# dohlee/metheor

Measured on AMD Instinct MI355X. Metric: M reads/sec (PDR+LPMD, 150bp WGBS), higher is better.
Workload: dtype u32; 1 GPU; S-chr19-10M (BASELINE config 2): 10000000 x 150bp reads/GPU, chr19 58.6 Mbp, 2.94 CpG calls/read, fused PDR+LPMD, reference CLI defaults; reads_per_gpu=10000000, cpg_calls_per_gpu=29424182, sites_emitted=726028, parallelism=contig-sharded x1

## Files before the change

### metheor_amd/build.py

```python
import hashlib
import json
import os
import shutil
import subprocess
import sys
import time

HERE = os.path.dirname(os.path.abspath(__file__))
CSRC = os.path.join(HERE, "csrc")
LIB = os.path.join(HERE, "libmetheor_hip.so")
ARCH = "gfx950"
HIP_FLAGS = os.environ.get("MTH_EXTRA_HIPFLAGS", "").split() + ["-O3", "-std=c++17", "-fPIC", "-Wall", "-ffp-contract=off", "-Wno-unused-result"]

HIP_SOURCES = ["mth_api.hip", "mth_pdr_lpmd.hip", "mth_pdr_wide.hip", "mth_quartet.hip", "mth_scan.hip", "mth_sites.hip", "mth_mhl_tile.hip", "mth_fdrp.hip", "mth_fdrp_wtile.hip", "mth_pairs.hip", "mth_decode.hip", "mth_sort.hip", "mth_fileorder.hip", "mth_inflate.hip", "mth_rccl.hip", "mth_tag.hip", "mth_multi.hip"]
HOST_LIB = os.path.join(HERE, "libmetheor_host.so")
HOST_SOURCES = [os.path.join("host", "bam_reader.cpp"), os.path.join("host", "host_api.cpp"),
                os.path.join("host", "parallel_decode.cpp"), os.path.join("host", "synth_bam.cpp"), os.path.join("host", "bai_index.cpp"), os.path.join("host", "sam_text.cpp")]
HOST_HEADERS = [os.path.join("host", "bam_reader.h"), os.path.join("host", "parallel_decode.h"), os.path.join("host", "bai_internal.h"), os.path.join("host", "sam_text.h"), os.path.join("..", "..", "include", "metheor_host.h")]
HEADERS = ["mth_common.h", "mth_ctx.h", "mth_quartet_dev.h", "mth_scan.h", "mth_tile_dev.h", "mth_wave_tile.h", os.path.join("..", "..", "include", "metheor_hip.h")]


def _hipcc():
    for c in (shutil.which("hipcc"), "/opt/rocm/bin/hipcc"):
        if c and os.path.exists(c):
            return c
    raise RuntimeError("hipcc not found: the engine is HIP-only (no CPU fallback)")


BUILD_INFO = os.path.join(HERE, "BUILD_INFO.json")


def _sha(path):
    with open(path, "rb") as f:
        return hashlib.sha256(f.read()).hexdigest()[:16]


def _stale(target, deps):
    if not os.path.exists(target):
        return True
    t = os.path.getmtime(target)
    return any(os.path.getmtime(d) > t for d in deps if os.path.exists(d))


def source_files():
    out = [os.path.join("csrc", s) for s in HIP_SOURCES + HEADERS + HOST_SOURCES + HOST_HEADERS] + [os.path.join("csrc", "host", "cli_main.cpp")]
    return sorted(set(os.path.normpath(p) for p in out))


def source_hashes():
    return {p: _sha(os.path.join(HERE, p)) for p in source_files()}


def _write_build_info(rebuilt):
    try:
        ver = subprocess.run([_hipcc(), "--version"], capture_output=True, text=True).stdout.splitlines()[0]
    except Exception:
        ver = "?"
    info = {"built_at": time.strftime("%Y-%m-%dT%H:%M:%SZ", time.gmtime()), "rebuilt_this_call": bool(rebuilt), "arch": ARCH, "hipcc": ver,
            "hip_flags": HIP_FLAGS, "artefacts": {os.path.basename(p): _sha(p) for p in (LIB, HOST_LIB, CLI) if os.path.exists(p)},
            "sources": source_hashes()}
    old = None
    if os.path.exists(BUILD_INFO):
        try:
            old = json.load(open(BUILD_INFO))
        except Exception:
            old = None
    if old and not rebuilt and old.get("sources") == info["sources"] and old.get("artefacts") == info["artefacts"]:
        return
    with open(BUILD_INFO, "w") as f:
        json.dump(info, f, indent=1, sort_keys=True)


# ... 72 lines not shown
```

### metheor_amd/csrc/mth_pdr_lpmd.hip

```cpp
#include "mth_ctx.h"
#include "mth_tile_dev.h"

#ifndef MTH_TILE_PF
#define MTH_TILE_PF 1
#endif

namespace mth {


constexpr int IDX_GROUPS = 1;
template <int NIDX>
__global__ __launch_bounds__(BLOCK) void k_build_index(const int32_t *__restrict__ read_start,
                                                       uint32_t n_reads, int32_t idx_base, int32_t idx_base2, int qshift,
                                                       uint32_t nq, int aligned16,
                                                       uint32_t *__restrict__ idx, uint32_t *__restrict__ idx2,
                                                       DevState *__restrict__ st, DevState *__restrict__ cst,
                                                       unsigned long long *__restrict__ bucket_sums, uint32_t n_bucket_words,
                                                       const uint32_t *__restrict__ cpg_off, uint32_t n_cpgs) {
    const uint32_t gtid = blockIdx.x * BLOCK + threadIdx.x;
    if (gtid == 0 && cst) cst->cur_base = cst->n_sites;
    for (uint32_t w = gtid; w < n_bucket_words; w += gridDim.x * BLOCK) bucket_sums[w] = 0ull;
    if (cpg_off && gtid < 64) {
        uint32_t best = 0;
#pragma unroll
// ... 266 lines not shown
    int32_t s = 0;
    uint32_t o0 = 0, n = 0, mq = 0;
    constexpr bool PF = MTH_TILE_PF && !CLAMP && sizeof(RelT) == 1 && NB == 8;
    uint32_t o1 = 0;
    if (PF) { if (i < hi) { o0 = a.cpg_off[i]; o1 = a.cpg_off[i + 1]; } }
    else if (i < hi) { s = a.read_start[i]; o0 = a.cpg_off[i]; n = a.cpg_off[i + 1] - o0; mq = a.read_mapq[i]; }
    while (i < hi) {
        const uint32_t inext = i + B;
        const bool more = inext < hi;
        uint32_t v[NB];
        int32_t r[NB];
        uint32_t rraw0 = 0, rraw1 = 0;
        uint32_t o0n = 0, o1n = 0;
        if constexpr (PF) {
            n = o1 - o0;
            const uint32_t *__restrict__ cp = a.cpg_pos + o0;
#pragma unroll
            for (int k4 = 0; k4 < NB / 4; ++k4) {
                const u32x4_a4 x = *reinterpret_cast<const u32x4_a4 *>(cp + 4 * k4);
                v[4 * k4] = x.x; v[4 * k4 + 1] = x.y; v[4 * k4 + 2] = x.z; v[4 * k4 + 3] = x.w;
            }
            if (do_lp) { const u32x2_a1 x = *reinterpret_cast<const u32x2_a1 *>(reinterpret_cast<const RelT *>(a.cpg_rel) + o0); rraw0 = x.x; rraw1 = x.y; }
            s = a.read_start[i]; mq = a.read_mapq[i];
            if (more) { o0n = a.cpg_off[inext]; o1n = a.cpg_off[inext + 1]; }
        }
        const bool owned = (s >= T0) && (s < T1);
        const bool lp_ok = do_lp && owned && (mq >= a.lpmd_min_qual);
        if (do_lp && owned) { n_read += 1; n_valid += lp_ok ? 1u : 0u; }
        const bool pdr_ok = a.want_pdr && (n >= a.min_cpgs) && (mq >= a.pdr_min_qual) && (n > 0);
        const bool work = (lp_ok || pdr_ok) && n != 0;
        const int32_t maxd = PACKED ? min(a.max_dist, 255) : min(a.max_dist, 1 << 20);
        const int32_t mind = max(a.min_dist, 0);
        const bool any_lp = maxd >= a.min_dist && maxd >= 0 && __any(work && lp_ok && n > 1);
        if (work) {
            const uint32_t *__restrict__ cp = a.cpg_pos + o0;
            const RelT *__restrict__ rp = rel + o0;
            if (PF) {
                (void)cp; (void)rp;
            } else if (!CLAMP) {
#pragma unroll
                for (int k4 = 0; k4 < NB / 4; ++k4) {
                    const u32x4_a4 x = *reinterpret_cast<const u32x4_a4 *>(cp + 4 * k4);
                    v[4 * k4] = x.x; v[4 * k4 + 1] = x.y; v[4 * k4 + 2] = x.z; v[4 * k4 + 3] = x.w;
                }
                if (any_lp) {
                    if constexpr (PACKED) { const u32x2_a1 x = *reinterpret_cast<const u32x2_a1 *>(rp); rraw0 = x.x; rraw1 = x.y; }
                    else load_rel<RelT, NB>(rp, r);
                }
            } else {
#pragma unroll
                for (int k = 0; k < NB; ++k) v[k] = cp[min((uint32_t)k, n - 1)];
                if (any_lp) {
#pragma unroll
                    for (int k = 0; k < NB; ++k) r[k] = (int32_t)rp[min((uint32_t)k, n - 1)];
                }
            }
        const uint32_t sm1 = (uint32_t)(s - 1);
        const uint32_t dead_w = ((MARGIN ? (uint32_t)(P0 - MG + (tid & 63)) : (uint32_t)T0 + (1u << 28)) & 0x7fffffffu) | (v[0] & 0x80000000u);
        const uint32_t n_lp = lp_ok ? min(n, (uint32_t)NB) : 0u;
        uint32_t acc = 0, xmax = (v[0] & 0x7fffffffu) - sm1;
        if constexpr (PACKED) {
            const uint32_t nrow = min(n, 8u);
            const uint4 ma = reinterpret_cast<const uint4 *>(&tabs.mtab[nrow][0])[0], mb = reinterpret_cast<const uint4 *>(&tabs.mtab[nrow][0])[1];
            const uint32_t mk[8] = {ma.x, ma.y, ma.z, ma.w, mb.x, mb.y, mb.z, mb.w};
            uint32_t xs[8];
            xs[0] = xmax;
#pragma unroll
            for (int k = 1; k < 8; ++k) {
                xs[k] = __builtin_amdgcn_bitop3_b32(v[k] - sm1, mk[k], 0x7fffffffu, 0x80);
                v[k] = __builtin_amdgcn_bitop3_b32(v[k], dead_w, mk[k], 0xe4);
                acc = __builtin_amdgcn_bitop3_b32(acc, v[k], v[0], 0xf6);
            }
            xmax = max(max(max(xs[0], xs[1]), max(xs[2], xs[3])), max(max(xs[4], xs[5]), max(xs[6], xs[7])));
        } else {
#pragma unroll
            for (int k = 1; k < NB; ++k) {
                const bool live = (uint32_t)k < n;
                const uint32_t x = (v[k] & 0x7fffffffu) - sm1;
                xmax = max(xmax, live ? x : 0u);
                v[k] = live ? v[k] : dead_w;
                acc |= v[k] ^ v[0];
            }
            if (any_lp) {
#pragma unroll
                for (int k = 0; k < NB; ++k) r[k] = ((uint32_t)k < n_lp) ? r[k] : (int32_t)((k + 1) << 24);
            }
        }
        uint32_t bad_it = (xmax > (uint32_t)a.max_span) ? 1u : 0u;
        uint32_t disc = acc >> 31;
        const bool any_long = __any(n > (uint32_t)NB);
        if (any_long && n > (uint32_t)NB) {
            const uint32_t first = v[0] >> 31;
            for (uint32_t k = NB; k < n; ++k) {
                const uint32_t x = a.cpg_pos[o0 + k];
                disc |= (x >> 31) ^ first;
                bad_it |= ((x & 0x7fffffffu) - sm1 > (uint32_t)a.max_span) ? 1u : 0u;
            }
        }
        bad |= bad_it;
        if constexpr (PACKED) {
            if (any_lp) {
                uint32_t SQ[4], SO[4], Q[4], O[4];
#pragma unroll
                for (int e = 0; e < 4; ++e) SQ[e] = __builtin_amdgcn_perm(v[2 * e + 1], v[2 * e], 0x070c030cu);
#pragma unroll
                for (int e = 0; e < 3; ++e) SO[e] = __builtin_amdgcn_perm(v[2 * e + 2], v[2 * e + 1], 0x070c030cu);
                SO[3] = __builtin_amdgcn_perm(0u, v[7], 0x070c030cu);
                if (!CLAMP) {
                    Q[0] = __builtin_amdgcn_perm(0u, rraw0, 0x0c010c00u); Q[1] = __builtin_amdgcn_perm(0u, rraw0, 0x0c030c02u);
                    Q[2] = __builtin_amdgcn_perm(0u, rraw1, 0x0c010c00u); Q[3] = __builtin_amdgcn_perm(0u, rraw1, 0x0c030c02u);
                    O[0] = __builtin_amdgcn_perm(0u, rraw0, 0x0c020c01u); O[1] = __builtin_amdgcn_perm(rraw1, rraw0, 0x0c040c03u);
                    O[2] = __builtin_amdgcn_perm(0u, rraw1, 0x0c020c01u); O[3] = __builtin_amdgcn_perm(0u, rraw1, 0x0c0c0c03u);
                } else {
#pragma unroll
                    for (int e = 0; e < 4; ++e) Q[e] = (uint32_t)r[2 * e] | ((uint32_t)r[2 * e + 1] << 16);
#pragma unroll
                    for (int e = 0; e < 3; ++e) O[e] = (uint32_t)r[2 * e + 1] | ((uint32_t)r[2 * e + 2] << 16);
                    O[3] = (uint32_t)r[7];
                }
                {
                    const uint4 da = reinterpret_cast<const uint4 *>(&tabs.dtab[n_lp][0])[0], db = reinterpret_cast<const uint4 *>(&tabs.dtab[n_lp][0])[1];
                    Q[0] += da.x; Q[1] += da.y; Q[2] += da.z; Q[3] += da.w; O[0] += db.x; O[1] += db.y; O[2] += db.z; O[3] += db.w;
                }
                const uint32_t KA = (0x8000u - (uint32_t)mind) * 0x10001u, KB = (0x8000u + (uint32_t)maxd) * 0x10001u;
                uint32_t accIN = 0, accDD = 0;
#pragma unroll
                for (int g = 1; g < 8; ++g) {
                    uint32_t orB = 0;
#pragma unroll
                    for (int m = 0; m < 4; ++m) {
                        const int li = (g & 1) ? (g - 1) / 2 + m : g / 2 + m;
                        if (li > 3) break;
                        const uint32_t later = (g & 1) ? O[li] : Q[li], sl = (g & 1) ? SO[li] : SQ[li];
                        const uint32_t D = later - Q[m];
                        const uint32_t Bw = KB - D;
                        const uint32_t IN = __builtin_amdgcn_bitop3_b32(D + KA, Bw, 0x80008000u, 0x80);
                        const uint32_t DD = IN & (sl ^ SQ[m]);
                        accIN += __builtin_popcount(IN);
                        accDD += __builtin_popcount(DD);
                        orB |= Bw;
                    }
                    if (!__any((orB & 0x80008000u) != 0u)) break;
                }
                lp_c += accIN - accDD;
                lp_d += accDD;
            }
        } else if (any_lp) {
            const uint32_t span_ok = (uint32_t)(maxd - a.min_dist);
            uint32_t lp_n = 0, lp_dd = 0;
#pragma unroll
            for (int g = 1; g < NB; ++g) {
                int32_t dmin = 0x7fffffff;
#pragma unroll
                for (int k = g; k < NB; ++k) {
                    const int32_t dist = r[k] - r[k - g];
                    dmin = min(dmin, dist);
                    const bool in = (uint32_t)(dist - a.min_dist) <= span_ok;
                    lp_n += in ? 1u : 0u;
                    lp_dd += (in ? (v[k] ^ v[k - g]) : 0u) >> 31;
                }
                if (!__any(dmin <= maxd)) break;
            }
            lp_c += lp_n - lp_dd;
            lp_d += lp_dd;
        }
        if (any_long && lp_ok && n > (uint32_t)NB) {
            for (uint32_t k = NB; k < n; ++k) {
                const int32_t rk = (int32_t)rel[o0 + k];
                const uint32_t mk = a.cpg_pos[o0 + k] >> 31;
                for (uint32_t j = k; j-- > 0;) {
                    const int32_t dist = rk - (int32_t)rel[o0 + j];
                    if (dist > a.max_dist) break;
                    if (dist < a.min_dist) continue;
                    if ((a.cpg_pos[o0 + j] >> 31) == mk) lp_c += 1; else lp_d += 1;
                }
            }
        }
        if (MARGIN) {
            if (pdr_ok && !bad_it && (uint32_t)s - (uint32_t)(P0 - MG + 1) <= (uint32_t)(W + MG - 1)) {
                const uint32_t one = disc ? 0x10001u : 1u;
                const uint32_t base4 = (uint32_t)(P0 - MG) << 2;
#pragma unroll
                for (int k = 0; k < NB; ++k)
                    atomicAdd(reinterpret_cast<uint32_t *>(reinterpret_cast<char *>(cnt_raw) + ((v[k] << 2) - base4)), one);
                if (any_long) {
                    for (uint32_t k = NB; k < n; ++k) {
                        const uint32_t pk = (a.cpg_pos[o0 + k] & 0x7fffffffu) - (uint32_t)P0;
                        if (pk < Wp) atomicAdd(cnt + pk, one);
                    }
                }
            }
        } else if (!WIDE) {
            const uint32_t one = disc ? 0x10001u : 1u;
            const uint32_t base4 = ((uint32_t)P0 << 2) - (pdr_ok ? 0u : (1u << 30));
            const uint32_t trash4 = (uint32_t)(W + (tid & 63)) << 2;
#pragma unroll
            for (int k = 0; k < NB; ++k) {
                const uint32_t a4 = min((v[k] << 2) - base4, trash4);
                atomicAdd(reinterpret_cast<uint32_t *>(reinterpret_cast<char *>(cnt) + a4), one);
// ... 189 lines not shown
        w = MTH_RUNS_MAP == 1 ? x * cpx + j : x * cpx + (j & 31u) * k + (j >> 5);
    }
    [[maybe_unused]] const unsigned long long rt_beg = RT_NOW();
    [[maybe_unused]] unsigned long long rt_loop = 0, rt_b1 = 0, rt_comp = 0, rt_b2 = 0, rt_pre = 0, rt_t = rt_beg, rt_ntile = 0, rt_wait = 0, rt_iters = 0;
    for (int i = tid; i < W / 4; i += B) reinterpret_cast<uint4 *>(cnt)[i] = make_uint4(0, 0, 0, 0);
    slot_tabs_init(tabs, tid);
    if (tid < 2) { s_lon[tid] = 0; s_more[tid] = 0; }
    if (tid < 4) s_rows[tid] = 0;
    if (tid < 16) s_lp[tid >> 2][tid & 3] = 0ull;
    if (w == 0 && tid == 0 && ra.cst) ra.cst->cur_base = ra.cst->n_sites;

    const uint32_t r0 = (uint32_t)(((unsigned long long)w * nr) / G), r1 = (uint32_t)(((unsigned long long)(w + 1u) * nr) / G);
    auto tile_of = [&](uint32_t r) -> uint32_t {
        const int64_t d = (int64_t)a.read_start[r] - a.region_beg;
        return d <= 0 ? 0u : (uint32_t)min((int64_t)ntiles, d / W);
    };
    const uint32_t tb = __builtin_amdgcn_readfirstlane((w == 0 || nr == 0) ? 0u : tile_of(r0));
    const uint32_t te = __builtin_amdgcn_readfirstlane((w + 1u == G || nr == 0) ? ntiles : max(tb, tile_of(r1)));
    {
        uint32_t err = 0;
        const uint32_t vend = min(r1 + 1u, nr);
        auto check4 = [&](const u32x4_a4 x, int32_t pv, uint32_t i0) {
            const int32_t e0 = (int32_t)x.x, e1 = (int32_t)x.y, e2 = (int32_t)x.z, e3 = (int32_t)x.w;
            if (i0 < vend) err |= e0 < pv ? 1u : 0u;
            if (i0 + 1u < vend) err |= e1 < e0 ? 1u : 0u;
            if (i0 + 2u < vend) err |= e2 < e1 ? 1u : 0u;
            if (i0 + 3u < vend) err |= e3 < e2 ? 1u : 0u;
        };
        constexpr int VSTEPS = 8;
        u32x4_a4 vx[VSTEPS]; int32_t vp[VSTEPS];
#pragma unroll
        for (int j = 0; j < VSTEPS; ++j) {
            const uint32_t i0 = r0 + 1u + 4u * ((uint32_t)tid + 256u * (uint32_t)j);
            vx[j] = u32x4_a4{0, 0, 0, 0}; vp[j] = 0;
            if (i0 < vend) {
                vp[j] = a.read_start[i0 - 1u];
                if (i0 + 4u <= nr) vx[j] = *reinterpret_cast<const u32x4_a4 *>(a.read_start + i0);
                else { vx[j].x = (uint32_t)a.read_start[i0]; vx[j].y = i0 + 1u < nr ? (uint32_t)a.read_start[i0 + 1u] : 0u; vx[j].z = i0 + 2u < nr ? (uint32_t)a.read_start[i0 + 2u] : 0u; vx[j].w = 0u; }
            }
        }
#pragma unroll
        for (int j = 0; j < VSTEPS; ++j) check4(vx[j], vp[j], r0 + 1u + 4u * ((uint32_t)tid + 256u * (uint32_t)j));
        for (uint32_t i = r0 + 1u + 1024u * VSTEPS + (uint32_t)tid; i < vend; i += B) err |= a.read_start[i] < a.read_start[i - 1u] ? 1u : 0u;
        if (err) atomicOr(const_cast<uint32_t *>(&a.st->err), (uint32_t)ERRB_UNSORTED);
    }
    if (tid == 0) { ra.run_tile0[w] = tb; if (w + 1u == G) ra.run_tile0[G] = ntiles; }

    const __amdgpu_buffer_rsrc_t rs_pos = __builtin_amdgcn_make_buffer_rsrc(const_cast<uint32_t *>(a.cpg_pos), 0, a.n_cpgs * 4u, 0x00020000);
    const __amdgpu_buffer_rsrc_t rs_rel = __builtin_amdgcn_make_buffer_rsrc(const_cast<void *>(a.cpg_rel), 0, a.n_cpgs, 0x00020000);
    const bool do_lp = a.want_lpmd != 0;
    const int32_t maxd = min(a.max_dist, 255);
    const int32_t mind = max(a.min_dist, 0);
    const bool lp_range = maxd >= a.min_dist && maxd >= 0;
    const uint32_t KA = (0x8000u - (uint32_t)mind) * 0x10001u, KB = (0x8000u + (uint32_t)maxd) * 0x10001u;

    uint32_t lp_c = 0, lp_d = 0, nrv = 0;
    auto flush_lpmd = [&]() {
        const unsigned long long f0 = wave_sum64(lp_c), f1 = wave_sum64(lp_d), f2 = wave_sum64(nrv & 0x7fffu), f3 = wave_sum64((nrv >> 15) & 0x7fffu);
        if (lane == 0) { s_lp[wave][0] += f0; s_lp[wave][1] += f1; s_lp[wave][2] += f2; s_lp[wave][3] += f3; }
        lp_c = lp_d = 0; nrv &= 0x80000000u;
    };

    uint32_t t = tb;
    uint32_t lo = 0;
    if (t < te) {
        const int32_t T0 = a.region_beg + (int32_t)(t * W);
        lo = __builtin_amdgcn_readfirstlane(wave_lower_bound(a.read_start, nr, (int32_t)max((int64_t)T0 - a.max_span + 1, (int64_t)INT32_MIN), r0, ra.hint_stride));
    }
    __syncthreads();
    uint32_t par = 0;
    uint32_t i = 0, o0 = 0, o1 = 0;
    int32_t s = INT32_MAX;
    auto fetch = [&](uint32_t idx) {
        i = idx; s = INT32_MAX; o0 = 0; o1 = 0;
        if (idx < nr) { s = a.read_start[idx]; o0 = a.cpg_off[idx]; o1 = a.cpg_off[idx + 1u]; }
    };
    int32_t s_first = INT32_MAX;
    if (t < te) { fetch(lo + (uint32_t)tid); s_first = __builtin_amdgcn_readfirstlane(lo < nr ? a.read_start[lo] : INT32_MAX); }
    uint32_t lon_run = 0;

    RT_ADD(rt_pre, rt_t);
    while (t < te) {
        const int32_t T0 = a.region_beg + (int32_t)(t * W);
        const int64_t T0W = (int64_t)T0 + W;
        const int32_t T1 = (int32_t)min(T0W, (int64_t)a.region_end);
        const uint32_t Wp = (uint32_t)(T1 - T0);
        const int32_t P0 = T0;
        if ((int64_t)s_first > T0W) {
            uint32_t tnext = te;
            if (lo < nr) tnext = (uint32_t)min((int64_t)te, max((int64_t)t + 1, ((int64_t)s_first - a.region_beg + W - 1) / W - 1));
            if (a.want_pdr) for (uint32_t q = 4u * t + (uint32_t)tid; q < 4u * tnext; q += B) a.tile_cnt[q] = 0u;
            t = tnext;
            continue;
        }
        const int32_t cmax = (int32_t)min(T0W, (int64_t)INT32_MAX);
        const int32_t nb = (int32_t)max(T0W - a.max_span + 1, (int64_t)INT32_MIN);
        bool first = true, last;
        do {
            uint32_t below_end = 0;
            uint32_t it = 0;
            bool cand = s <= cmax;
            while (it < PT_PASS_ITERS && __any(cand)) {
                uint32_t v[NB];
                const uint32_t n = o1 - o0;
#ifdef MTH_RUNS_GLOBAL_LOADS
                {
                    const u32x4_a4 x0 = *reinterpret_cast<const u32x4_a4 *>(a.cpg_pos + o0);
// ... 21 lines not shown
                {
                    const unsigned long long bm = __ballot(cand && s < nb);
                    if (bm) below_end = max(below_end, i - (uint32_t)lane + 64u - (uint32_t)__builtin_clzll(bm));
                }
                const bool owned = cand && (s >= T0) && (s < T1);
                const bool lp_ok = do_lp && owned && (mq >= a.lpmd_min_qual);
                if (do_lp && owned) nrv += lp_ok ? 0x8001u : 1u;
                const bool pdr_ok = cand && a.want_pdr && (n >= a.min_cpgs) && (mq >= a.pdr_min_qual) && (n > 0);
                const bool work = (lp_ok || pdr_ok) && n != 0;
                const bool any_lp = lp_range && __any(work && lp_ok && n > 1);
                if (work) {
                    const uint32_t sm1 = (uint32_t)(s - 1);
                    const uint32_t dead_w = ((MARGIN ? (uint32_t)(P0 - MG + lane) : (uint32_t)T0 + (1u << 28)) & 0x7fffffffu) | (v[0] & 0x80000000u);
                    const uint32_t n_lp = lp_ok ? min(n, (uint32_t)NB) : 0u;
                    uint32_t acc = 0, xmax;
                    {
                        const uint32_t nrow = min(n, 8u);
                        const uint4 ma = reinterpret_cast<const uint4 *>(&tabs.mtab[nrow][0])[0], mb = reinterpret_cast<const uint4 *>(&tabs.mtab[nrow][0])[1];
                        const uint32_t mk[8] = {ma.x, ma.y, ma.z, ma.w, mb.x, mb.y, mb.z, mb.w};
                        uint32_t xs[8];
                        xs[0] = (v[0] & 0x7fffffffu) - sm1;
#pragma unroll
                        for (int k = 1; k < 8; ++k) {
                            xs[k] = __builtin_amdgcn_bitop3_b32(v[k] - sm1, mk[k], 0x7fffffffu, 0x80);
                            v[k] = __builtin_amdgcn_bitop3_b32(v[k], dead_w, mk[k], 0xe4);
                            acc = __builtin_amdgcn_bitop3_b32(acc, v[k], v[0], 0xf6);
                        }
                        xmax = max(max(max(xs[0], xs[1]), max(xs[2], xs[3])), max(max(xs[4], xs[5]), max(xs[6], xs[7])));
                    }
                    uint32_t bad_it = (xmax > (uint32_t)a.max_span) ? 1u : 0u;
                    uint32_t disc = acc >> 31;
                    const bool any_long = __any(n > (uint32_t)NB);
                    if (any_long && n > (uint32_t)NB) {
                        const uint32_t firstst = v[0] >> 31;
                        for (uint32_t k = NB; k < n; ++k) {
                            const uint32_t x = a.cpg_pos[o0 + k];
                            disc |= (x >> 31) ^ firstst;
                            bad_it |= ((x & 0x7fffffffu) - sm1 > (uint32_t)a.max_span) ? 1u : 0u;
                        }
                    }
                    nrv |= bad_it << 31;
                    if (any_lp) {
                        if (__any(o0 + 8u > a.n_cpgs)) {
                            if (o0 + 8u > a.n_cpgs) {
                                const uint8_t *__restrict__ rel = reinterpret_cast<const uint8_t *>(a.cpg_rel);
                                rraw0 = rraw1 = 0;
#pragma unroll 1
                                for (uint32_t k = 0; k < 8u && o0 + k < a.n_cpgs; ++k) {
                                    const uint32_t bte = rel[o0 + k];
                                    if (k < 4) rraw0 |= bte << (8 * k); else rraw1 |= bte << (8 * (k - 4));
                                }
                            }
                        }
                        uint32_t SQ[4], SO[4], Q[4], O[4];
#pragma unroll
                        for (int e = 0; e < 4; ++e) SQ[e] = __builtin_amdgcn_perm(v[2 * e + 1], v[2 * e], 0x070c030cu);
#pragma unroll
                        for (int e = 0; e < 3; ++e) SO[e] = __builtin_amdgcn_perm(v[2 * e + 2], v[2 * e + 1], 0x070c030cu);
                        SO[3] = __builtin_amdgcn_perm(0u, v[7], 0x070c030cu);
                        Q[0] = __builtin_amdgcn_perm(0u, rraw0, 0x0c010c00u); Q[1] = __builtin_amdgcn_perm(0u, rraw0, 0x0c030c02u);
                        Q[2] = __builtin_amdgcn_perm(0u, rraw1, 0x0c010c00u); Q[3] = __builtin_amdgcn_perm(0u, rraw1, 0x0c030c02u);
                        O[0] = __builtin_amdgcn_perm(0u, rraw0, 0x0c020c01u); O[1] = __builtin_amdgcn_perm(rraw1, rraw0, 0x0c040c03u);
                        O[2] = __builtin_amdgcn_perm(0u, rraw1, 0x0c020c01u); O[3] = __builtin_amdgcn_perm(0u, rraw1, 0x0c0c0c03u);
                        {
                            const uint4 da = reinterpret_cast<const uint4 *>(&tabs.dtab[n_lp][0])[0], db = reinterpret_cast<const uint4 *>(&tabs.dtab[n_lp][0])[1];
                            Q[0] += da.x; Q[1] += da.y; Q[2] += da.z; Q[3] += da.w; O[0] += db.x; O[1] += db.y; O[2] += db.z; O[3] += db.w;
                        }
                        uint32_t accIN = 0, accDD = 0;
#pragma unroll
                        for (int g = 1; g < 8; ++g) {
                            uint32_t orB = 0;
#pragma unroll
                            for (int m = 0; m < 4; ++m) {
                                const int li = (g & 1) ? (g - 1) / 2 + m : g / 2 + m;
                                if (li > 3) break;
                                const uint32_t later = (g & 1) ? O[li] : Q[li], sl = (g & 1) ? SO[li] : SQ[li];
                                const uint32_t D = later - Q[m];
                                const uint32_t Bw = KB - D;
                                const uint32_t IN = __builtin_amdgcn_bitop3_b32(D + KA, Bw, 0x80008000u, 0x80);
                                const uint32_t DD = IN & (sl ^ SQ[m]);
                                accIN += __builtin_popcount(IN);
                                accDD += __builtin_popcount(DD);
                                orB |= Bw;
                            }
                            if (!__any((orB & 0x80008000u) != 0u)) break;
                        }
                        lp_c += accIN - accDD;
                        lp_d += accDD;
                    }
                    if (any_long && lp_ok && n > (uint32_t)NB) {
                        const uint8_t *__restrict__ rel = reinterpret_cast<const uint8_t *>(a.cpg_rel);
                        for (uint32_t k = NB; k < n; ++k) {
                            const int32_t rk = (int32_t)rel[o0 + k];
                            const uint32_t mk = a.cpg_pos[o0 + k] >> 31;
                            for (uint32_t j = k; j-- > 0;) {
                                const int32_t dist = rk - (int32_t)rel[o0 + j];
                                if (dist > a.max_dist) break;
                                if (dist < a.min_dist) continue;
                                if ((a.cpg_pos[o0 + j] >> 31) == mk) lp_c += 1; else lp_d += 1;
                            }
                        }
                    }
                    if (MARGIN) {
                        if (pdr_ok && !bad_it && (uint32_t)s - (uint32_t)(P0 - MG + 1) <= (uint32_t)(W + MG - 1)) {
                            const uint32_t one = disc ? 0x10001u : 1u;
                            const uint32_t base4 = (uint32_t)(P0 - MG) << 2;
#pragma unroll
                            for (int k = 0; k < NB; ++k)
                                atomicAdd(reinterpret_cast<uint32_t *>(reinterpret_cast<char *>(cnt_raw) + ((v[k] << 2) - base4)), one);
                            if (any_long) {
                                for (uint32_t k = NB; k < n; ++k) {
                                    const uint32_t pk = (a.cpg_pos[o0 + k] & 0x7fffffffu) - (uint32_t)P0;
                                    if (pk < Wp) atomicAdd(cnt + pk, one);
                                }
                            }
                        }
                    } else {
                        const uint32_t one = disc ? 0x10001u : 1u;
                        const uint32_t base4 = ((uint32_t)P0 << 2) - (pdr_ok ? 0u : (1u << 30));
                        const uint32_t trash4 = (uint32_t)(W + lane) << 2;
#pragma unroll
                        for (int k = 0; k < NB; ++k) {
                            const uint32_t a4 = min((v[k] << 2) - base4, trash4);
                            atomicAdd(reinterpret_cast<uint32_t *>(reinterpret_cast<char *>(cnt) + a4), one);
                        }
                        if (any_long && pdr_ok) {
                            for (uint32_t k = NB; k < n; ++k) {
                                const uint32_t pk = (a.cpg_pos[o0 + k] & 0x7fffffffu) - (uint32_t)P0;
                                if (pk < Wp) atomicAdd(cnt + pk, one);
                            }
                        }
                    }
                }
                i = inx; s = sn; o0 = o0n; o1 = o1n;
                cand = s <= cmax;
                ++it;
            }
            const bool more_w = __any(cand);
            if (lane == 0) {
                if (below_end) atomicMax(&s_lon[par], below_end);
                if (more_w) s_more[par] = 1u;
// ... 593 lines not shown
```

### metheor_amd/csrc/mth_pdr_wide.hip

```cpp
#include "mth_ctx.h"
#include "mth_quartet_dev.h"
#include "mth_tile_dev.h"

namespace mth {

#ifndef MTH_PW_QCAP
#define MTH_PW_QCAP 3072
#endif
#ifndef MTH_PW_OCC
#define MTH_PW_OCC 7
#endif
constexpr int PW_S = 1024, PW_B = 256, PW_U = 2, PW_NB = 8, PW_QCAP = MTH_PW_QCAP;
constexpr uint32_t PW_EMPTY = 0xffffffffu;
constexpr int FQ_S = 512, FQ_OCC = 4, FQ_QCAP = 2048;

template <int SHIFT, typename RelT, bool QUARTET, int QCAP>
__device__ __forceinline__ void tile_pass(const TileArgs &a, const FusedQuartet &q, const uint32_t ntiles) {
    constexpr int W = 1 << SHIFT;
    constexpr bool PACKED = sizeof(RelT) == 1;
    __shared__ uint32_t tkey[PW_S], tcov[PW_S], tdisc[PW_S];
    __shared__ uint32_t bcnt[PW_B];
    __shared__ uint32_t q_or_sort[QCAP / 2];
    static_assert(QCAP / 2 >= PW_B, "bbase fits under the queue");
    uint16_t *const rq = reinterpret_cast<uint16_t *>(q_or_sort);
// ... 103 lines not shown
                static_assert(PW_NB == 8, "two 16-byte loads per read");
                if (__all(!act || (unsigned long long)o0 + PW_NB <= (unsigned long long)a.n_cpgs)) {
                    if (act) {
                        const u32x4_a4 x = *reinterpret_cast<const u32x4_a4 *>(a.cpg_pos + o0), y = *reinterpret_cast<const u32x4_a4 *>(a.cpg_pos + o0 + 4);
                        v[0] = x.x; v[1] = x.y; v[2] = x.z; v[3] = x.w; v[4] = y.x; v[5] = y.y; v[6] = y.z; v[7] = y.w;
                        if constexpr (PACKED) { const u32x2_a1 z = *reinterpret_cast<const u32x2_a1 *>(rel + o0); rraw0 = z.x; rraw1 = z.y; }
                        else {
                            const u32x4_a2 z = *reinterpret_cast<const u32x4_a2 *>(rel + o0);
                            r[0] = (int32_t)(z.x & 0xffffu); r[1] = (int32_t)(z.x >> 16); r[2] = (int32_t)(z.y & 0xffffu); r[3] = (int32_t)(z.y >> 16);
                            r[4] = (int32_t)(z.z & 0xffffu); r[5] = (int32_t)(z.z >> 16); r[6] = (int32_t)(z.w & 0xffffu); r[7] = (int32_t)(z.w >> 16);
                        }
                    }
                } else if (act) {
#pragma unroll
                    for (int k = 0; k < PW_NB; ++k) {
                        const uint32_t kk = o0 + min((uint32_t)k, n - 1);
                        v[k] = a.cpg_pos[kk];
                        const uint32_t rv = (uint32_t)rel[kk];
                        if constexpr (PACKED) { if (k < 4) rraw0 |= rv << (8 * k); else rraw1 |= rv << (8 * (k - 4)); }
                        else r[k] = (int32_t)rv;
                    }
                }
                const int32_t s = a.read_start[i];
                const uint32_t mq = a.read_mapq[i];
                const bool owned = act && s >= P0 && s < P1;
                const bool lp_ok = lp_possible && owned && mq >= a.lpmd_min_qual && n > 1;
                const bool pdr_ok = act && a.want_pdr && n >= a.min_cpgs && mq >= a.pdr_min_qual;
                const uint32_t sm1 = (uint32_t)(s - 1);
                const uint32_t nrow = min(n, 8u);
                const uint4 ma = reinterpret_cast<const uint4 *>(&tabs.mtab[nrow][0])[0], mb = reinterpret_cast<const uint4 *>(&tabs.mtab[nrow][0])[1];
                const uint32_t mk[8] = {ma.x, ma.y, ma.z, ma.w, mb.x, mb.y, mb.z, mb.w};
                uint32_t acc = 0, xmax = act ? (v[0] & 0x7fffffffu) - sm1 : 0u;
#pragma unroll
                for (int k = 1; k < PW_NB; ++k) {
                    xmax = max(xmax, __builtin_amdgcn_bitop3_b32(v[k] - sm1, mk[k], 0x7fffffffu, 0x80));
                    v[k] = __builtin_amdgcn_bitop3_b32(v[k], v[0], mk[k], 0xe4);
                    acc |= v[k] ^ v[0];
                }
                uint32_t bad_it = (xmax > (uint32_t)a.max_span) ? 1u : 0u;
                uint32_t disc = acc >> 31;
                const bool any_long = __any(n > (uint32_t)PW_NB);
                if (any_long && n > (uint32_t)PW_NB) {
                    const uint32_t first = v[0] >> 31;
                    for (uint32_t k = PW_NB; k < n; ++k) {
                        const uint32_t x = a.cpg_pos[o0 + k];
                        disc |= (x >> 31) ^ first;
                        bad_it |= ((x & 0x7fffffffu) - sm1 > (uint32_t)a.max_span) ? 1u : 0u;
                    }
                }
                bad |= act ? bad_it : 0u;
                if (__any(lp_ok)) {
                    const uint32_t n_lp = lp_ok ? min(n, (uint32_t)PW_NB) : 0u;
                    if constexpr (PACKED) {
                        uint32_t SQ[4], SO[4], Q[4], O[4];
#pragma unroll
                        for (int e = 0; e < 4; ++e) SQ[e] = __builtin_amdgcn_perm(v[2 * e + 1], v[2 * e], 0x070c030cu);
#pragma unroll
                        for (int e = 0; e < 3; ++e) SO[e] = __builtin_amdgcn_perm(v[2 * e + 2], v[2 * e + 1], 0x070c030cu);
                        SO[3] = __builtin_amdgcn_perm(0u, v[7], 0x070c030cu);
                        Q[0] = __builtin_amdgcn_perm(0u, rraw0, 0x0c010c00u); Q[1] = __builtin_amdgcn_perm(0u, rraw0, 0x0c030c02u);
                        Q[2] = __builtin_amdgcn_perm(0u, rraw1, 0x0c010c00u); Q[3] = __builtin_amdgcn_perm(0u, rraw1, 0x0c030c02u);
                        O[0] = __builtin_amdgcn_perm(0u, rraw0, 0x0c020c01u); O[1] = __builtin_amdgcn_perm(rraw1, rraw0, 0x0c040c03u);
                        O[2] = __builtin_amdgcn_perm(0u, rraw1, 0x0c020c01u); O[3] = __builtin_amdgcn_perm(0u, rraw1, 0x0c0c0c03u);
                        {
                            const uint4 da = reinterpret_cast<const uint4 *>(&tabs.dtab[n_lp][0])[0], db = reinterpret_cast<const uint4 *>(&tabs.dtab[n_lp][0])[1];
                            Q[0] += da.x; Q[1] += da.y; Q[2] += da.z; Q[3] += da.w; O[0] += db.x; O[1] += db.y; O[2] += db.z; O[3] += db.w;
                        }
                        const uint32_t KA = (0x8000u - (uint32_t)mind) * 0x10001u, KB = (0x8000u + (uint32_t)maxd) * 0x10001u;
                        uint32_t accIN = 0, accDD = 0;
#pragma unroll
                        for (int g = 1; g < 8; ++g) {
                            uint32_t orB = 0;
#pragma unroll
                            for (int m = 0; m < 4; ++m) {
                                const int li = (g & 1) ? (g - 1) / 2 + m : g / 2 + m;
                                if (li > 3) break;
                                const uint32_t later = (g & 1) ? O[li] : Q[li], sl = (g & 1) ? SO[li] : SQ[li];
                                const uint32_t D = later - Q[m];
                                const uint32_t Bw = KB - D;
                                const uint32_t IN = __builtin_amdgcn_bitop3_b32(D + KA, Bw, 0x80008000u, 0x80);
                                const uint32_t DD = IN & (sl ^ SQ[m]);
                                accIN += __builtin_popcount(IN);
                                accDD += __builtin_popcount(DD);
                                orB |= Bw;
                            }
                            if (!__any((orB & 0x80008000u) != 0u)) break;
                        }
                        a_c += accIN - accDD;
                        a_d += accDD;
                    } else {
#pragma unroll
                        for (int k = 0; k < PW_NB; ++k) r[k] = ((uint32_t)k < n_lp) ? r[k] : (int32_t)((k + 1) << 24);
                        const uint32_t span_ok = (uint32_t)(maxd - a.min_dist);
                        uint32_t lp_n = 0, lp_dd = 0;
#pragma unroll
                        for (int g = 1; g < PW_NB; ++g) {
                            int32_t dmin = 0x7fffffff;
#pragma unroll
                            for (int k = g; k < PW_NB; ++k) {
                                const int32_t dist = r[k] - r[k - g];
                                dmin = min(dmin, dist);
                                const bool in = (uint32_t)(dist - a.min_dist) <= span_ok;
                                lp_n += in ? 1u : 0u;
                                lp_dd += (in ? (v[k] ^ v[k - g]) : 0u) >> 31;
                            }
                            if (!__any(dmin <= maxd)) break;
                        }
                        a_c += lp_n - lp_dd;
                        a_d += lp_dd;
                    }
                    if (any_long && lp_ok && n > (uint32_t)PW_NB) {
                        for (uint32_t k = PW_NB; k < n; ++k) {
                            const int32_t rk = (int32_t)rel[o0 + k];
                            const uint32_t mkk = a.cpg_pos[o0 + k] >> 31;
                            for (uint32_t jj = k; jj-- > 0;) {
                                const int32_t dist = rk - (int32_t)rel[o0 + jj];
                                if (dist > a.max_dist) break;
                                if (dist < a.min_dist) continue;
                                if ((a.cpg_pos[o0 + jj] >> 31) == mkk) a_c += 1; else a_d += 1;
                            }
                        }
                    }
                }
                if (__any(pdr_ok && !bad_it)) {
                    auto insert = [&](const uint32_t word) {
                        const uint32_t p = word & 0x7fffffffu, d = p - (uint32_t)P0;
                        if (d >= Wp) return;
                        uint32_t h = (d >> 1) & (PW_S - 1), probes = 0;
                        while (probes++ < (uint32_t)PW_S) {
                            const uint32_t cur = atomicCAS(&tkey[h], PW_EMPTY, p);
                            if (cur == PW_EMPTY || cur == p) { atomicAdd(&tcov[h], 1u); if (disc) atomicAdd(&tdisc[h], 1u); return; }
                            h = (h + 1) & (PW_S - 1);
                        }
                        s_over = 1u;
                    };
                    const bool go = pdr_ok && !bad_it;
#pragma unroll
                    for (int k = 0; k < PW_NB; ++k) {
                        if (!__any(go && (uint32_t)k < n)) break;
                        if (go && (uint32_t)k < n) insert(v[k]);
                    }
                    if (any_long && go && n > (uint32_t)PW_NB)
// ... 132 lines not shown
```

### metheor_amd/csrc/mth_tile_dev.h

```cpp
#pragma once
#include "mth_common.h"

namespace mth {

#define MTH_DPP(v, ctrl, rmask, bctl) ((uint32_t)__builtin_amdgcn_update_dpp(0, (int)(v), (ctrl), (rmask), 0xf, (bctl)))
__device__ __forceinline__ uint32_t wave_sum(uint32_t v) {
    v += MTH_DPP(v, 0xb1 , 0xf, true);
    v += MTH_DPP(v, 0x4e , 0xf, true);
    v += MTH_DPP(v, 0x141 , 0xf, true);
    v += MTH_DPP(v, 0x140 , 0xf, true);
    return __builtin_amdgcn_readlane(v, 0) + __builtin_amdgcn_readlane(v, 16) + __builtin_amdgcn_readlane(v, 32) +
           __builtin_amdgcn_readlane(v, 48);
}
__device__ __forceinline__ uint32_t wave_scan_incl(uint32_t v) {
    v += MTH_DPP(v, 0x111 , 0xf, true);
    v += MTH_DPP(v, 0x112 , 0xf, true);
    v += MTH_DPP(v, 0x114 , 0xf, true);
    v += MTH_DPP(v, 0x118 , 0xf, true);
    v += MTH_DPP(v, 0x142 , 0xa, false);
    v += MTH_DPP(v, 0x143 , 0xc, false);
    return v;
}

constexpr int TILE_BUCKET_SHIFT = 8;

struct TileArgs {
    const int32_t  *read_start;
    const uint8_t  *read_mapq;
    const uint32_t *cpg_off;
    const uint32_t *cpg_pos;
    const void     *cpg_rel;
    const uint32_t *idx;
    const uint32_t *idx2;
    const DevState *st;
    uint32_t *tile_cnt;
    unsigned long long *bucket;
    uint32_t nbk;
    SiteRec  *scratch;
    int32_t region_beg, region_end, idx_base, max_span;
    uint32_t n_reads, n_cpgs;
    uint32_t min_cov;
    uint32_t min_cpgs;
    int32_t  min_dist, max_dist;
    uint8_t  pdr_min_qual, lpmd_min_qual, want_pdr, want_lpmd;
    uint32_t tile_w_rt;
#ifdef MTH_TILE_TRACE
    unsigned long long *trace;
#endif
};

typedef uint32_t u32x4_a4 __attribute__((ext_vector_type(4), aligned(4)));
typedef uint32_t u32x2_a1 __attribute__((ext_vector_type(2), aligned(1)));
typedef uint32_t u32x4_a2 __attribute__((ext_vector_type(4), aligned(2)));

void launch_tile_wide(const TileArgs &a, uint32_t ntiles, int shift, bool rel8, hipStream_t s);

struct FusedQuartet {
    uint8_t force;
    uint8_t force_heavy;
    uint8_t min_qual;
    unsigned long long *qs;
    unsigned long long row_cap;
    uint32_t max_tiles;
    uint32_t *tile_flag;
    unsigned long long *tile_row0;
    uint32_t *tile_rows;
    int32_t *out_pos; uint32_t *out_cnt; float *out_me, *out_pm; uint32_t *out_depth;
    bool taken;
    uint32_t ntiles;
};
void launch_tile_fused(const TileArgs &a, const FusedQuartet &q, uint32_t ntiles, int shift, bool rel8, hipStream_t s);

struct SlotTabs {
    uint32_t mtab[9][8];
    uint32_t dtab[9][8];
};
__device__ __forceinline__ void slot_tabs_init(SlotTabs &T, const int tid) {
    if (tid < 72) {
        const uint32_t nn = (uint32_t)tid >> 3, c = (uint32_t)tid & 7u;
        T.mtab[nn][c] = c < nn ? 0xffffffffu : 0u;
        auto dead = [&](uint32_t k) { return k >= 8u ? 0x2400u : (k >= nn ? 0x400u * (k + 1u) : 0u); };
        const uint32_t lo = c < 4 ? 2u * c : 2u * (c - 4u) + 1u;
        T.dtab[nn][c] = dead(lo) | (dead(lo + 1u) << 16);
    }
}
__device__ __forceinline__ uint32_t bfi(uint32_t mask, uint32_t a, uint32_t b) { return (a & mask) | (b & ~mask); }


}
```

Baseline: 113,900 M reads/s.

## Evaluate LPMD pair distances in packed 8-bit SWAR lanes instead of 16-bit fields

Adds a byte-packed SWAR path for the LPMD pairwise distance test. When min and max distance fit in 7 bits, each 32-bit word holds four relative positions and four state bits, and each lag is processed with alignbyte/bitop3/popcount, with a shared-memory per-count validity mask table. This halves the words handled per lag compared with the 16-bit field version, which is kept as a fallback and now deduplicated into one helper used by three kernels. The cost is extra shared-memory table space, a runtime domain branch, and a second lane-pair pass for short lags.

```diff
diff --git a/metheor_amd/build.py b/metheor_amd/build.py
--- a/metheor_amd/build.py
+++ b/metheor_amd/build.py
@@ -17,7 +17,7 @@
 HOST_SOURCES = [os.path.join("host", "bam_reader.cpp"), os.path.join("host", "host_api.cpp"),
                 os.path.join("host", "parallel_decode.cpp"), os.path.join("host", "synth_bam.cpp"), os.path.join("host", "bai_index.cpp"), os.path.join("host", "sam_text.cpp")]
 HOST_HEADERS = [os.path.join("host", "bam_reader.h"), os.path.join("host", "parallel_decode.h"), os.path.join("host", "bai_internal.h"), os.path.join("host", "sam_text.h"), os.path.join("..", "..", "include", "metheor_host.h")]
-HEADERS = ["mth_common.h", "mth_ctx.h", "mth_quartet_dev.h", "mth_scan.h", "mth_tile_dev.h", "mth_wave_tile.h", os.path.join("..", "..", "include", "metheor_hip.h")]
+HEADERS = ["mth_common.h", "mth_ctx.h", "mth_quartet_dev.h", "mth_scan.h", "mth_tile_dev.h", "mth_lpmd_bytes.h", "mth_wave_tile.h", os.path.join("..", "..", "include", "metheor_hip.h")]
 
 
 def _hipcc():
diff --git a/metheor_amd/csrc/mth_lpmd_bytes.h b/metheor_amd/csrc/mth_lpmd_bytes.h
--- /dev/null
+++ b/metheor_amd/csrc/mth_lpmd_bytes.h
@@ -0,0 +1,100 @@
+#pragma once
+#include <stdint.h>
+
+#if defined(__HIPCC__)
+#define MTH_LB_FN __host__ __device__ __forceinline__
+#else
+#define MTH_LB_FN inline
+#endif
+
+namespace mth {
+
+MTH_LB_FN bool lpmd_bytes_domain(const int32_t mind, const int32_t maxd) { return mind >= 0 && mind <= 128 && maxd >= 0 && maxd <= 127; }
+
+struct alignas(8) LpMask { uint32_t w0, w1; };
+
+MTH_LB_FN uint32_t lpmd_bytes_mask(const uint32_t n, const uint32_t g, const uint32_t w) {
+    uint32_t m = 0;
+    for (uint32_t j = 0; j < 4; ++j) m |= (4u * w + j + g < n) ? 0x80u << (8u * j) : 0u;
+    return m;
+}
+
+MTH_LB_FN uint32_t lb_alignbyte(const uint32_t hi, const uint32_t lo, const int sh) {
+#if defined(__HIP_DEVICE_COMPILE__)
+    return __builtin_amdgcn_alignbyte(hi, lo, (uint32_t)sh);
+#else
+    return (uint32_t)((((uint64_t)hi << 32) | lo) >> (8 * sh));
+#endif
+}
+MTH_LB_FN uint32_t lb_perm(const uint32_t a, const uint32_t b, const uint32_t sel) {
+#if defined(__HIP_DEVICE_COMPILE__)
+    return __builtin_amdgcn_perm(a, b, sel);
+#else
+    uint32_t r = 0;
+    for (int k = 0; k < 4; ++k) {
+        const uint32_t s = (sel >> (8 * k)) & 0xffu;
+        const uint32_t byte = s < 4 ? (b >> (8 * s)) & 0xffu : (s < 8 ? (a >> (8 * (s - 4))) & 0xffu : 0u);
+        r |= byte << (8 * k);
+    }
+    return r;
+#endif
+}
+template <int TT>
+MTH_LB_FN uint32_t lb_bitop3(const uint32_t a, const uint32_t b, const uint32_t c) {
+#if defined(__HIP_DEVICE_COMPILE__)
+    return __builtin_amdgcn_bitop3_b32(a, b, c, TT);
+#else
+    uint32_t r = 0;
+    for (int i = 0; i < 8; ++i)
+        if ((TT >> i) & 1) r |= ((i & 4) ? a : ~a) & ((i & 2) ? b : ~b) & ((i & 1) ? c : ~c);
+    return r;
+#endif
+}
+MTH_LB_FN bool lb_any(const bool x) {
+#if defined(__HIP_DEVICE_COMPILE__)
+    return __any(x);
+#else
+    return x;
+#endif
+}
+
+MTH_LB_FN uint32_t lpmd_state_bytes(const uint32_t v0, const uint32_t v1, const uint32_t v2, const uint32_t v3) {
+    return lb_perm(v1, v0, 0x0c0c0703u) | lb_perm(v3, v2, 0x07030c0cu);
+}
+
+MTH_LB_FN void lpmd_pairs_bytes(const uint32_t E0, const uint32_t E1, const uint32_t S0, const uint32_t S1, const LpMask *mrow,
+                                const uint32_t mind, const uint32_t maxd, uint32_t &lp_c, uint32_t &lp_d) {
+    const uint32_t KA = (0x80u - mind) * 0x01010101u, KB = (0x80u + maxd) * 0x01010101u;
+    uint32_t accIN = 0, accDD = 0;
+#pragma unroll
+    for (int g = 1; g < 8; ++g) {
+        const LpMask m = mrow[g];
+        uint32_t orY;
+        {
+            const uint32_t L = g < 4 ? lb_alignbyte(E1, E0, g) : E1 >> (8 * (g & 3));
+            const uint32_t SL = g < 4 ? lb_alignbyte(S1, S0, g) : S1 >> (8 * (g & 3));
+            const uint32_t D = L - E0;
+            const uint32_t d7 = D & 0x7f7f7f7fu;
+            const uint32_t Y = lb_bitop3<0x20>(KB - d7, D, m.w0);
+            const uint32_t IN = (d7 + KA) & Y;
+            accIN += (uint32_t)__builtin_popcount(IN);
+            accDD += (uint32_t)__builtin_popcount(lb_bitop3<0x60>(IN, SL, S0));
+            orY = Y;
+        }
+        if (g < 4 && lb_any(m.w1 != 0u)) {
+            const uint32_t L = E1 >> (8 * g), SL = S1 >> (8 * g);
+            const uint32_t D = L - E1;
+            const uint32_t d7 = D & 0x7f7f7f7fu;
+            const uint32_t Y = lb_bitop3<0x20>(KB - d7, D, m.w1);
+            const uint32_t IN = (d7 + KA) & Y;
+            accIN += (uint32_t)__builtin_popcount(IN);
+            accDD += (uint32_t)__builtin_popcount(lb_bitop3<0x60>(IN, SL, S1));
+            orY |= Y;
+        }
+        if (!lb_any(orY != 0u)) break;
+    }
+    lp_c += accIN - accDD;
+    lp_d += accDD;
+}
+
+}
diff --git a/metheor_amd/csrc/mth_pdr_lpmd.hip b/metheor_amd/csrc/mth_pdr_lpmd.hip
--- a/metheor_amd/csrc/mth_pdr_lpmd.hip
+++ b/metheor_amd/csrc/mth_pdr_lpmd.hip
@@ -342,7 +342,11 @@
                 for (int k = 0; k < NB; ++k) v[k] = cp[min((uint32_t)k, n - 1)];
                 if (any_lp) {
 #pragma unroll
-                    for (int k = 0; k < NB; ++k) r[k] = (int32_t)rp[min((uint32_t)k, n - 1)];
+                    for (int k = 0; k < NB; ++k) {
+                        const uint32_t rv = (uint32_t)rp[min((uint32_t)k, n - 1)];
+                        if constexpr (PACKED) { if (k < 4) rraw0 |= rv << (8 * k); else rraw1 |= rv << (8 * (k - 4)); }
+                        else r[k] = (int32_t)rv;
+                    }
                 }
             }
         const uint32_t sm1 = (uint32_t)(s - 1);
@@ -389,52 +393,7 @@
         }
         bad |= bad_it;
         if constexpr (PACKED) {
-            if (any_lp) {
-                uint32_t SQ[4], SO[4], Q[4], O[4];
-#pragma unroll
-                for (int e = 0; e < 4; ++e) SQ[e] = __builtin_amdgcn_perm(v[2 * e + 1], v[2 * e], 0x070c030cu);
-#pragma unroll
-                for (int e = 0; e < 3; ++e) SO[e] = __builtin_amdgcn_perm(v[2 * e + 2], v[2 * e + 1], 0x070c030cu);
-                SO[3] = __builtin_amdgcn_perm(0u, v[7], 0x070c030cu);
-                if (!CLAMP) {
-                    Q[0] = __builtin_amdgcn_perm(0u, rraw0, 0x0c010c00u); Q[1] = __builtin_amdgcn_perm(0u, rraw0, 0x0c030c02u);
-                    Q[2] = __builtin_amdgcn_perm(0u, rraw1, 0x0c010c00u); Q[3] = __builtin_amdgcn_perm(0u, rraw1, 0x0c030c02u);
-                    O[0] = __builtin_amdgcn_perm(0u, rraw0, 0x0c020c01u); O[1] = __builtin_amdgcn_perm(rraw1, rraw0, 0x0c040c03u);
-                    O[2] = __builtin_amdgcn_perm(0u, rraw1, 0x0c020c01u); O[3] = __builtin_amdgcn_perm(0u, rraw1, 0x0c0c0c03u);
-                } else {
-#pragma unroll
-                    for (int e = 0; e < 4; ++e) Q[e] = (uint32_t)r[2 * e] | ((uint32_t)r[2 * e + 1] << 16);
-#pragma unroll
-                    for (int e = 0; e < 3; ++e) O[e] = (uint32_t)r[2 * e + 1] | ((uint32_t)r[2 * e + 2] << 16);
-                    O[3] = (uint32_t)r[7];
-                }
-                {
-                    const uint4 da = reinterpret_cast<const uint4 *>(&tabs.dtab[n_lp][0])[0], db = reinterpret_cast<const uint4 *>(&tabs.dtab[n_lp][0])[1];
-                    Q[0] += da.x; Q[1] += da.y; Q[2] += da.z; Q[3] += da.w; O[0] += db.x; O[1] += db.y; O[2] += db.z; O[3] += db.w;
-                }
-                const uint32_t KA = (0x8000u - (uint32_t)mind) * 0x10001u, KB = (0x8000u + (uint32_t)maxd) * 0x10001u;
-                uint32_t accIN = 0, accDD = 0;
-#pragma unroll
-                for (int g = 1; g < 8; ++g) {
-                    uint32_t orB = 0;
-#pragma unroll
-                    for (int m = 0; m < 4; ++m) {
-                        const int li = (g & 1) ? (g - 1) / 2 + m : g / 2 + m;
-                        if (li > 3) break;
-                        const uint32_t later = (g & 1) ? O[li] : Q[li], sl = (g & 1) ? SO[li] : SQ[li];
-                        const uint32_t D = later - Q[m];
-                        const uint32_t Bw = KB - D;
-                        const uint32_t IN = __builtin_amdgcn_bitop3_b32(D + KA, Bw, 0x80008000u, 0x80);
-                        const uint32_t DD = IN & (sl ^ SQ[m]);
-                        accIN += __builtin_popcount(IN);
-                        accDD += __builtin_popcount(DD);
-                        orB |= Bw;
-                    }
-                    if (!__any((orB & 0x80008000u) != 0u)) break;
-                }
-                lp_c += accIN - accDD;
-                lp_d += accDD;
-            }
+            if (any_lp) lpmd_pairs8(v, rraw0, rraw1, n_lp, tabs, mind, maxd, lp_c, lp_d);
         } else if (any_lp) {
             const uint32_t span_ok = (uint32_t)(maxd - a.min_dist);
             uint32_t lp_n = 0, lp_dd = 0;
@@ -730,7 +689,6 @@
     const int32_t maxd = min(a.max_dist, 255);
     const int32_t mind = max(a.min_dist, 0);
     const bool lp_range = maxd >= a.min_dist && maxd >= 0;
-    const uint32_t KA = (0x8000u - (uint32_t)mind) * 0x10001u, KB = (0x8000u + (uint32_t)maxd) * 0x10001u;
 
     uint32_t lp_c = 0, lp_d = 0, nrv = 0;
     auto flush_lpmd = [&]() {
@@ -858,41 +816,7 @@
                                 }
                             }
                         }
-                        uint32_t SQ[4], SO[4], Q[4], O[4];
-#pragma unroll
-                        for (int e = 0; e < 4; ++e) SQ[e] = __builtin_amdgcn_perm(v[2 * e + 1], v[2 * e], 0x070c030cu);
-#pragma unroll
-                        for (int e = 0; e < 3; ++e) SO[e] = __builtin_amdgcn_perm(v[2 * e + 2], v[2 * e + 1], 0x070c030cu);
-                        SO[3] = __builtin_amdgcn_perm(0u, v[7], 0x070c030cu);
-                        Q[0] = __builtin_amdgcn_perm(0u, rraw0, 0x0c010c00u); Q[1] = __builtin_amdgcn_perm(0u, rraw0, 0x0c030c02u);
-                        Q[2] = __builtin_amdgcn_perm(0u, rraw1, 0x0c010c00u); Q[3] = __builtin_amdgcn_perm(0u, rraw1, 0x0c030c02u);
-                        O[0] = __builtin_amdgcn_perm(0u, rraw0, 0x0c020c01u); O[1] = __builtin_amdgcn_perm(rraw1, rraw0, 0x0c040c03u);
-                        O[2] = __builtin_amdgcn_perm(0u, rraw1, 0x0c020c01u); O[3] = __builtin_amdgcn_perm(0u, rraw1, 0x0c0c0c03u);
-                        {
-                            const uint4 da = reinterpret_cast<const uint4 *>(&tabs.dtab[n_lp][0])[0], db = reinterpret_cast<const uint4 *>(&tabs.dtab[n_lp][0])[1];
-                            Q[0] += da.x; Q[1] += da.y; Q[2] += da.z; Q[3] += da.w; O[0] += db.x; O[1] += db.y; O[2] += db.z; O[3] += db.w;
-                        }
-                        uint32_t accIN = 0, accDD = 0;
-#pragma unroll
-                        for (int g = 1; g < 8; ++g) {
-                            uint32_t orB = 0;
-#pragma unroll
-                            for (int m = 0; m < 4; ++m) {
-                                const int li = (g & 1) ? (g - 1) / 2 + m : g / 2 + m;
-                                if (li > 3) break;
-                                const uint32_t later = (g & 1) ? O[li] : Q[li], sl = (g & 1) ? SO[li] : SQ[li];
-                                const uint32_t D = later - Q[m];
-                                const uint32_t Bw = KB - D;
-                                const uint32_t IN = __builtin_amdgcn_bitop3_b32(D + KA, Bw, 0x80008000u, 0x80);
-                                const uint32_t DD = IN & (sl ^ SQ[m]);
-                                accIN += __builtin_popcount(IN);
-                                accDD += __builtin_popcount(DD);
-                                orB |= Bw;
-                            }
-                            if (!__any((orB & 0x80008000u) != 0u)) break;
-                        }
-                        lp_c += accIN - accDD;
-                        lp_d += accDD;
+                        lpmd_pairs8(v, rraw0, rraw1, n_lp, tabs, mind, maxd, lp_c, lp_d);
                     }
                     if (any_long && lp_ok && n > (uint32_t)NB) {
                         const uint8_t *__restrict__ rel = reinterpret_cast<const uint8_t *>(a.cpg_rel);
diff --git a/metheor_amd/csrc/mth_pdr_wide.hip b/metheor_amd/csrc/mth_pdr_wide.hip
--- a/metheor_amd/csrc/mth_pdr_wide.hip
+++ b/metheor_amd/csrc/mth_pdr_wide.hip
@@ -179,42 +179,7 @@
                 if (__any(lp_ok)) {
                     const uint32_t n_lp = lp_ok ? min(n, (uint32_t)PW_NB) : 0u;
                     if constexpr (PACKED) {
-                        uint32_t SQ[4], SO[4], Q[4], O[4];
-#pragma unroll
-                        for (int e = 0; e < 4; ++e) SQ[e] = __builtin_amdgcn_perm(v[2 * e + 1], v[2 * e], 0x070c030cu);
-#pragma unroll
-                        for (int e = 0; e < 3; ++e) SO[e] = __builtin_amdgcn_perm(v[2 * e + 2], v[2 * e + 1], 0x070c030cu);
-                        SO[3] = __builtin_amdgcn_perm(0u, v[7], 0x070c030cu);
-                        Q[0] = __builtin_amdgcn_perm(0u, rraw0, 0x0c010c00u); Q[1] = __builtin_amdgcn_perm(0u, rraw0, 0x0c030c02u);
-                        Q[2] = __builtin_amdgcn_perm(0u, rraw1, 0x0c010c00u); Q[3] = __builtin_amdgcn_perm(0u, rraw1, 0x0c030c02u);
-                        O[0] = __builtin_amdgcn_perm(0u, rraw0, 0x0c020c01u); O[1] = __builtin_amdgcn_perm(rraw1, rraw0, 0x0c040c03u);
-                        O[2] = __builtin_amdgcn_perm(0u, rraw1, 0x0c020c01u); O[3] = __builtin_amdgcn_perm(0u, rraw1, 0x0c0c0c03u);
-                        {
-                            const uint4 da = reinterpret_cast<const uint4 *>(&tabs.dtab[n_lp][0])[0], db = reinterpret_cast<const uint4 *>(&tabs.dtab[n_lp][0])[1];
-                            Q[0] += da.x; Q[1] += da.y; Q[2] += da.z; Q[3] += da.w; O[0] += db.x; O[1] += db.y; O[2] += db.z; O[3] += db.w;
-                        }
-                        const uint32_t KA = (0x8000u - (uint32_t)mind) * 0x10001u, KB = (0x8000u + (uint32_t)maxd) * 0x10001u;
-                        uint32_t accIN = 0, accDD = 0;
-#pragma unroll
-                        for (int g = 1; g < 8; ++g) {
-                            uint32_t orB = 0;
-#pragma unroll
-                            for (int m = 0; m < 4; ++m) {
-                                const int li = (g & 1) ? (g - 1) / 2 + m : g / 2 + m;
-                                if (li > 3) break;
-                                const uint32_t later = (g & 1) ? O[li] : Q[li], sl = (g & 1) ? SO[li] : SQ[li];
-                                const uint32_t D = later - Q[m];
-                                const uint32_t Bw = KB - D;
-                                const uint32_t IN = __builtin_amdgcn_bitop3_b32(D + KA, Bw, 0x80008000u, 0x80);
-                                const uint32_t DD = IN & (sl ^ SQ[m]);
-                                accIN += __builtin_popcount(IN);
-                                accDD += __builtin_popcount(DD);
-                                orB |= Bw;
-                            }
-                            if (!__any((orB & 0x80008000u) != 0u)) break;
-                        }
-                        a_c += accIN - accDD;
-                        a_d += accDD;
+                        lpmd_pairs8(v, rraw0, rraw1, n_lp, tabs, mind, maxd, a_c, a_d);
                     } else {
 #pragma unroll
                         for (int k = 0; k < PW_NB; ++k) r[k] = ((uint32_t)k < n_lp) ? r[k] : (int32_t)((k + 1) << 24);
diff --git a/metheor_amd/csrc/mth_tile_dev.h b/metheor_amd/csrc/mth_tile_dev.h
--- a/metheor_amd/csrc/mth_tile_dev.h
+++ b/metheor_amd/csrc/mth_tile_dev.h
@@ -1,5 +1,6 @@
 #pragma once
 #include "mth_common.h"
+#include "mth_lpmd_bytes.h"
 
 namespace mth {
 
@@ -74,8 +75,10 @@
 struct SlotTabs {
     uint32_t mtab[9][8];
     uint32_t dtab[9][8];
+    LpMask   m8[9][8];
 };
 __device__ __forceinline__ void slot_tabs_init(SlotTabs &T, const int tid) {
+    if (tid < 144) (&T.m8[0][0].w0)[tid] = lpmd_bytes_mask((uint32_t)tid >> 4, ((uint32_t)tid >> 1) & 7u, (uint32_t)tid & 1u);
     if (tid < 72) {
         const uint32_t nn = (uint32_t)tid >> 3, c = (uint32_t)tid & 7u;
         T.mtab[nn][c] = c < nn ? 0xffffffffu : 0u;
@@ -86,5 +89,54 @@
 }
 __device__ __forceinline__ uint32_t bfi(uint32_t mask, uint32_t a, uint32_t b) { return (a & mask) | (b & ~mask); }
 
+__device__ __forceinline__ void lpmd_pairs_fields16(const uint32_t (&v)[8], const uint32_t rraw0, const uint32_t rraw1, const uint32_t *drow,
+                                                    const uint32_t mind, const uint32_t maxd, uint32_t &lp_c, uint32_t &lp_d) {
+    uint32_t SQ[4], SO[4], Q[4], O[4];
+#pragma unroll
+    for (int e = 0; e < 4; ++e) SQ[e] = __builtin_amdgcn_perm(v[2 * e + 1], v[2 * e], 0x070c030cu);
+#pragma unroll
+    for (int e = 0; e < 3; ++e) SO[e] = __builtin_amdgcn_perm(v[2 * e + 2], v[2 * e + 1], 0x070c030cu);
+    SO[3] = __builtin_amdgcn_perm(0u, v[7], 0x070c030cu);
+    Q[0] = __builtin_amdgcn_perm(0u, rraw0, 0x0c010c00u); Q[1] = __builtin_amdgcn_perm(0u, rraw0, 0x0c030c02u);
+    Q[2] = __builtin_amdgcn_perm(0u, rraw1, 0x0c010c00u); Q[3] = __builtin_amdgcn_perm(0u, rraw1, 0x0c030c02u);
+    O[0] = __builtin_amdgcn_perm(0u, rraw0, 0x0c020c01u); O[1] = __builtin_amdgcn_perm(rraw1, rraw0, 0x0c040c03u);
+    O[2] = __builtin_amdgcn_perm(0u, rraw1, 0x0c020c01u); O[3] = __builtin_amdgcn_perm(0u, rraw1, 0x0c0c0c03u);
+    {
+        const uint4 da = reinterpret_cast<const uint4 *>(drow)[0], db = reinterpret_cast<const uint4 *>(drow)[1];
+        Q[0] += da.x; Q[1] += da.y; Q[2] += da.z; Q[3] += da.w; O[0] += db.x; O[1] += db.y; O[2] += db.z; O[3] += db.w;
+    }
+    const uint32_t KA = (0x8000u - mind) * 0x10001u, KB = (0x8000u + maxd) * 0x10001u;
+    uint32_t accIN = 0, accDD = 0;
+#pragma unroll
+    for (int g = 1; g < 8; ++g) {
+        uint32_t orB = 0;
+#pragma unroll
+        for (int m = 0; m < 4; ++m) {
+            const int li = (g & 1) ? (g - 1) / 2 + m : g / 2 + m;
+            if (li > 3) break;
+            const uint32_t later = (g & 1) ? O[li] : Q[li], sl = (g & 1) ? SO[li] : SQ[li];
+            const uint32_t D = later - Q[m];
+            const uint32_t Bw = KB - D;
+            const uint32_t IN = __builtin_amdgcn_bitop3_b32(D + KA, Bw, 0x80008000u, 0x80);
+            const uint32_t DD = IN & (sl ^ SQ[m]);
+            accIN += __builtin_popcount(IN);
+            accDD += __builtin_popcount(DD);
+            orB |= Bw;
+        }
+        if (!__any((orB & 0x80008000u) != 0u)) break;
+    }
+    lp_c += accIN - accDD;
+    lp_d += accDD;
+}
+
+__device__ __forceinline__ void lpmd_pairs8(const uint32_t (&v)[8], const uint32_t rraw0, const uint32_t rraw1, const uint32_t n_lp,
+                                            const SlotTabs &T, const int32_t mind, const int32_t maxd, uint32_t &lp_c, uint32_t &lp_d) {
+    if (lpmd_bytes_domain(mind, maxd))
+        lpmd_pairs_bytes(rraw0, rraw1, lpmd_state_bytes(v[0], v[1], v[2], v[3]), lpmd_state_bytes(v[4], v[5], v[6], v[7]), &T.m8[n_lp][0],
+                         (uint32_t)mind, (uint32_t)maxd, lp_c, lp_d);
+    else
+        lpmd_pairs_fields16(v, rraw0, rraw1, &T.dtab[n_lp][0], (uint32_t)mind, (uint32_t)maxd, lp_c, lp_d);
+}
+
 
 }
```

Measured after the change: 119,900 M reads/s, median of 6. +5.3%, better.
